# lrjconan/LanczosNetwork

Measured on NVIDIA H100. Metric: QM8 molecules/sec (forward), higher is better.
Workload: dtype f32

## Files before the change

lanczosnetwork_b200/csrc/spectral_conv_fused.cu:

```cuda
#include "tc_gemm.cuh"

namespace {

constexpr int KMAX = 32;
constexpr int GMAX = 32;
constexpr int RMAX = 128;
constexpr int EMAX = 16;
constexpr int FR = 8;

template <bool STAGE>
__global__ void __launch_bounds__(256)
graph_prepare_kernel(const float* __restrict__ L, const float* __restrict__ Q, int N, int E1, int K,
                     float* __restrict__ ell_val, uint8_t* __restrict__ ell_idx,
                     int32_t* __restrict__ ell_max, int32_t* __restrict__ gext, int binarize) {
  extern __shared__ __align__(16) float gp_smem[];
  __shared__ int s_max[EMAX];
  __shared__ int s_ext[2];
  __shared__ uint8_t cnt_s[256 * EMAX];
  const int b = blockIdx.x, tid = threadIdx.x;
  if (tid < EMAX) s_max[tid] = 0;
  if (tid < 2) s_ext[tid] = 0;
  const int64_t per = (int64_t)N * N * E1;
  const float* Lg = L + b * per;
  if (STAGE) {
// ... 476 lines not shown
  float* ring;
  tcg::PhaseTimer* ptm = nullptr;

  static __host__ __device__ constexpr size_t tables_bytes() { return (sizeof(Tables) + 15) & ~size_t(15); }

  __device__ SpectralPolicyT(const Params& p_, uint8_t* smem, int tid_)
      : p(p_), tid(tid_), r(tid_ & 127), N(p_.N), K(p_.K), S(p_.S), E1(p_.E1),
        H(p_.H), XP(x_pitch(p_.Din[0], p_.H)), Din(p_.Din[0]) {
    tb = reinterpret_cast<Tables*>(smem);
    Xs = reinterpret_cast<float*>(smem + tables_bytes());
    Qs = Xs + (size_t)RMAX * XP;
    Ev = Qs + (size_t)RMAX * K;
    Ei = reinterpret_cast<uint8_t*>(Ev + (size_t)p.LB * RMAX);
    ring = reinterpret_cast<float*>(tcg::a_ring(smem, kStagesB, kStagesA));
  }
  static size_t smem_fixed(int Din, int K, int H) {
    return (size_t)RMAX * x_pitch(Din, H) * 4 + (size_t)RMAX * K * 4 + tables_bytes() + 16;
  }
  static size_t ell_line_bytes() { return (size_t)RMAX * 5; }
  static size_t readout_bytes(int H, int P, int N) {
    const size_t P1 = (size_t)P + 1, PQ = (P1 + 3) / 4, yr = (RMAX + 1) * P1;
    return (4 * PQ * (H + 4) + yr + ((4 - (yr & 3)) & 3) + H) * 4 + (size_t)GMAX * N;
  }

  __device__ void build_tables(int m_tile) {
    const int lane = tid & 31;
    const int32_t* sc = schedule(p);
    const int s0 = __ldg(sc + 1 + m_tile), s1 = __ldg(sc + 2 + m_tile);
    const int ng = s1 - s0;
    int g = s0 + lane, n = 0, k = 0;
    if (lane < ng) {
      if (p.B >= 2) g = __ldg(sc + __ldg(sc) + 2 + s0 + lane);
      n = __ldg(p.gext + g * 2);
      k = __ldg(p.gext + g * 2 + 1);
    }
    const int nq = (n + 3) >> 2, kq = (k + 3) >> 2;
    int pn = n, pk = k, pq = nq, pz = kq;
#pragma unroll
    for (int o = 1; o < 32; o <<= 1) {
      const int a = __shfl_up_sync(0xffffffffu, pn, o), bq = __shfl_up_sync(0xffffffffu, pk, o);
      const int c = __shfl_up_sync(0xffffffffu, pq, o), d = __shfl_up_sync(0xffffffffu, pz, o);
      if (lane >= o) { pn += a; pk += bq; pq += c; pz += d; }
    }
    const int nb = pn - n, kb = pk - k, qb = pq - nq, zb = pz - kq;
    if (lane < ng) {
      tb->gid[lane] = g;
      tb->nbase[lane] = nb; tb->kbase[lane] = kb; tb->gn[lane] = n; tb->gk[lane] = k;
      for (int i = 0; i < n; ++i) { tb->row_g[nb + i] = (uint8_t)lane; tb->row_n[nb + i] = (uint8_t)i; }
      for (int i = 0; i < k; ++i) { tb->z_g[kb + i] = (uint8_t)lane; tb->z_k[kb + i] = (uint8_t)i; }
      for (int i = 0; i < nq; ++i) { tb->q_g[qb + i] = (uint8_t)lane; tb->q_n0[qb + i] = (uint8_t)(4 * i); }
      for (int i = 0; i < kq; ++i) { tb->zq_g[zb + i] = (uint8_t)lane; tb->zq_k0[zb + i] = (uint8_t)(4 * i); }
    }
    const int Rtot = __shfl_sync(0xffffffffu, pn, 31), Ztot = __shfl_sync(0xffffffffu, pk, 31);
    const int nquads = __shfl_sync(0xffffffffu, pq, 31), nzquads = __shfl_sync(0xffffffffu, pz, 31);
    int em[EMAX];
#pragma unroll
    for (int e = 0; e < EMAX; ++e)
      em[e] = (e < E1 && lane < ng) ? __ldg(p.ell_max + g * E1 + e) : 0;
#pragma unroll
    for (int e = 0; e < EMAX; ++e) {
      if (e < E1) {
        int m = em[e];
        if (lane < ng) tb->emax[lane][e] = (uint8_t)m;
#pragma unroll
        for (int o = 16; o > 0; o >>= 1) m = max(m, __shfl_xor_sync(0xffffffffu, m, o));
        if (lane == 0) tb->tmax_e[e] = m;
      }
    }
    __syncwarp();
    if (lane == 0) {
      tb->ng = ng; tb->Rtot = Rtot; tb->Ztot = Ztot; tb->nquads = nquads; tb->nzquads = nzquads;
      tb->nbase[ng] = Rtot; tb->kbase[ng] = Ztot;
      int left = p.LB, base = 0;
      for (int e = 0; e < E1; ++e) {
        const int c = min(tb->tmax_e[e], left);
        tb->cnt_e[e] = c; tb->base_e[e] = base;
        for (int t = 0; t < c; ++t) { tb->line_e[base + t] = (uint8_t)e; tb->line_t[base + t] = (uint8_t)t; }
        base += c; left -= c;
      }
      tb->nlines = base;
    }
  }

  __device__ void step_begin(int m_tile, int sub, int , tcg::PhaseTimer& tm) {
    tcg::producers_sync();
    const int layer = sub >> 1, step = sub & 1;
    if (step == 1 && S > 0) return;
    Din = p.Din[layer];
    const int warp = tid >> 5, lane = tid & 31;
    constexpr int NW = tcg::PRODUCER_THREADS / 32;
    const int dv = Din / 4;
    ptm = &tm;
    if (layer == 0) {
    if (warp == 0) build_tables(m_tile);
    tcg::producers_sync();
    tm.lap(16);
    const int Rtot = tb->Rtot;
    int64_t my_id = 0;
    if (!p.X && warp + lane * NW < Rtot) {
      const int row = warp + lane * NW;
      my_id = __ldg(p.node_ids + (int64_t)tb->gid[tb->row_g[row]] * N + tb->row_n[row]);
    }
    for (int row = warp, j = 0; row < Rtot; row += NW, ++j) {
      const int64_t src_row = (int64_t)tb->gid[tb->row_g[row]] * N + tb->row_n[row];
      const float* xsrc;
      if (p.X) {
        xsrc = p.X + src_row * Din;
      } else {
        int64_t id = __shfl_sync(0xffffffffu, my_id, j);
        id = id < 0 ? 0 : (id >= p.emb_rows ? p.emb_rows - 1 : id);
        xsrc = p.emb + id * Din;
      }
      float* xd = Xs + (size_t)row * XP;
      for (int q4 = lane; q4 < dv; q4 += 32) sm90::cp_async_16(xd + 4 * q4, xsrc + 4 * q4);
      const float* qsrc = p.Q + src_row * K;
      float* qd = Qs + (size_t)row * K;
      for (int k4 = lane; k4 < (K >> 2); k4 += 32) sm90::cp_async_16(qd + 4 * k4, qsrc + 4 * k4);
    }
    tm.lap(17);
    {
      constexpr int ELL_BATCH = 4;
      const int nlines = tb->nlines;
      for (int base = warp; base < nlines; base += NW * ELL_BATCH) {
        for (int r0 = 0; r0 < Rtot; r0 += 32) {
          const int rr = r0 + lane;
          float vv[ELL_BATCH];
          int ii[ELL_BATCH];
#pragma unroll
          for (int u = 0; u < ELL_BATCH; ++u) {
            const int line = base + u * NW;
            vv[u] = 0.f; ii[u] = 0;
            if (line < nlines && rr < Rtot) {
              const int e = tb->line_e[line], t = tb->line_t[line];
              const int g = tb->row_g[rr], n = tb->row_n[rr];
              if (t < tb->emax[g][e]) {
                const int64_t off = (((int64_t)tb->gid[g] * E1 + e) * N + t) * N + n;
                vv[u] = __ldg(p.ell_val + off);
                ii[u] = tb->nbase[g] + __ldg(p.ell_idx + off);
              }
            }
          }
#pragma unroll
          for (int u = 0; u < ELL_BATCH; ++u) {
            const int line = base + u * NW;
            if (line < nlines && rr < Rtot) {
              Ev[(size_t)line * RMAX + rr] = vv[u];
              Ei[(size_t)line * RMAX + rr] = (uint8_t)ii[u];
            }
          }
        }
      }
    }
    tm.lap(18);
    }
    const int Ztot = tb->Ztot;
#pragma unroll
    for (int i = 0; i < FR; ++i) fr[i] = 0.f;
    if (S > 0 && r < Ztot) {
      const float* f = p.coeff + layer * p.coeff_stride + ((int64_t)tb->gid[tb->z_g[r]] * K + tb->z_k[r]) * S;
#pragma unroll
      for (int i = 0; i < FR; ++i)
        if (i < S) fr[i] = __ldg(f + i);
    }
    tm.lap(0);
    sm90::cp_async_wait_all();
    tcg::producers_sync();
    tm.lap(1);
  }

  __device__ __forceinline__ void produce(int sub, int kb, float (&v)[32]) {
#pragma unroll
    for (int j = 0; j < 32; ++j) v[j] = 0.f;
    if (kLongScales && (sub & 1) == 0) {
      if (r >= tb->Ztot) return;
      const int s = kb % S;
      if (s == 0) {
        const int g = tb->z_g[r], n_g = tb->gn[g], nb = tb->nbase[g];
        const float* xs = Xs + (size_t)nb * XP + (kb / S) * tcg::BK;
        const float* qs = Qs + (size_t)nb * K + tb->z_k[r];
#pragma unroll
        for (int j = 0; j < tcg::BK; ++j) u[j] = 0.f;
#pragma unroll 2
        for (int n = 0; n < n_g; ++n) {
          const float q = qs[(size_t)n * K];
          const float4* x4 = reinterpret_cast<const float4*>(xs + (size_t)n * XP);
#pragma unroll
          for (int j = 0; j < 8; ++j) {
            const float4 t = x4[j];
            u[4 * j + 0] = fmaf(q, t.x, u[4 * j + 0]); u[4 * j + 1] = fmaf(q, t.y, u[4 * j + 1]);
            u[4 * j + 2] = fmaf(q, t.z, u[4 * j + 2]); u[4 * j + 3] = fmaf(q, t.w, u[4 * j + 3]);
          }
        }
      }
      float f = 0.f;
      if (S <= FR) {
#pragma unroll
        for (int i = 0; i < FR; ++i) f = (i == s) ? fr[i] : f;
      } else {
        f = __ldg(p.coeff + (sub >> 1) * p.coeff_stride + ((int64_t)tb->gid[tb->z_g[r]] * K + tb->z_k[r]) * S + s);
      }
#pragma unroll
      for (int j = 0; j < tcg::BK; ++j) v[j] = f * u[j];
      return;
    }
    const int j0 = kb * tcg::BK;
    const int c = j0 / Din, d0 = j0 - c * Din;
    if (r >= tb->Rtot) return;
    const int e = c;
    if constexpr (kMaxAgg) {
      produce_max(e, d0, v);
      return;
    }
    const float* xs = Xs + d0;
    const int ts = tb->cnt_e[e], tmax = tb->tmax_e[e];
    const float* ev = Ev + (size_t)tb->base_e[e] * RMAX + r;
    const uint8_t* ei = Ei + (size_t)tb->base_e[e] * RMAX + r;
#pragma unroll 2
    for (int t = 0; t < ts; ++t) {
      const float a = ev[t * RMAX];
      if (a == 0.f) continue;
      const int i = ei[t * RMAX];
      const float4* x4 = reinterpret_cast<const float4*>(xs + (size_t)i * XP);
#pragma unroll
      for (int q = 0; q < 8; ++q) {
        const float4 tt = x4[q];
        v[4 * q + 0] = fmaf(a, tt.x, v[4 * q + 0]);
        v[4 * q + 1] = fmaf(a, tt.y, v[4 * q + 1]);
        v[4 * q + 2] = fmaf(a, tt.z, v[4 * q + 2]);
        v[4 * q + 3] = fmaf(a, tt.w, v[4 * q + 3]);
      }
    }
    if (ts < tmax) {
      const int g = tb->row_g[r], n = tb->row_n[r];
      const int my = tb->emax[g][e], nb = tb->nbase[g];
      const int64_t off0 = (((int64_t)tb->gid[g] * E1 + e) * N) * N + n;
// ... 410 lines not shown
```

lanczosnetwork_b200/csrc/filter_mlp_chain.cu:

```cuda
#include "tc_gemm.cuh"

namespace {

constexpr int S0MAX = 8;

struct ChainPolicy {
  static constexpr int kStagesB = 2;
  static constexpr int kStagesA = 4;
  struct Params {
    const float* table;
    const int32_t* rowmap;
    const int32_t* nrows;
    const float* W_hi;
    const float* W_lo;
    const float* bias_all;
    float* coeff;
    int Rall, L, S, Hd;
    int dbg;
  };
  static __device__ __forceinline__ bool mma0(const Params& p) { return p.S > S0MAX; }
  static __device__ __forceinline__ int first_stage(const Params& p) { return mma0(p) ? 0 : 1; }
  static __device__ __forceinline__ int steps_per_item(const Params& p) { return mma0(p) ? 4 : 2; }
  static __device__ __forceinline__ int rows(const Params& p) { return p.nrows ? __ldg(p.nrows) : p.Rall; }
  static __device__ __forceinline__ int ntile(const Params& p) { return (rows(p) + tcg::BM - 1) / tcg::BM; }
  static __device__ __forceinline__ void item_range(const Params& p, int cta, int ncta, int& first,
                                                    int& count) {
    const int items = ntile(p) * p.L, base = items / ncta, rem = items % ncta;
    count = base + (cta < rem ? 1 : 0);
    first = cta * base + min(cta, rem);
  }
  static __device__ __forceinline__ int num_steps(const Params& p, int cta, int ncta) {
    int first, count;
    item_range(p, cta, ncta, first, count);
    return count * steps_per_item(p);
  }
  static __device__ __forceinline__ void decode(const Params& p, int cta, int ncta, int it,
                                                int& m_tile, int& sub) {
    const int per = steps_per_item(p), nt = ntile(p);
    int first, count;
    item_range(p, cta, ncta, first, count);
    const int item = first + it / per;
    m_tile = item % nt;
    sub = (item / nt) * 4 + first_stage(p) + it % per;
  }
  static __device__ __forceinline__ int num_kblocks(const Params& p, int sub) {
    return (sub & 3) == 0 ? 1 : p.Hd / tcg::BK;
  }
  static __device__ __forceinline__ int w_row0(const Params& p, int layer, int stage) {
    return layer * (3 * p.Hd + p.S) + stage * p.Hd;
  }
  static __device__ __forceinline__ void w_coords(const Params& p, int sub, int kb, int& col0, int& row0) {
    col0 = kb * tcg::BK;
    row0 = w_row0(p, sub >> 2, sub & 3);
  }
  static __device__ __forceinline__ bool operand_from_acc(const Params& p, int sub) {
    return (sub & 3) > first_stage(p);
  }
  static __device__ __forceinline__ float acc_operand(const Params&, const uint8_t* policy_smem, int sub, int col,
                                                      float x) {
    const float* bs = reinterpret_cast<const float*>(policy_smem) + BS_OFF;
    return fmaxf(x + bs[(sub & 3) * tcg::BN + col], 0.f);
  }

  const Params& p;
  const int tid, r;
  static constexpr int BS_OFF = 2 * tcg::BN * S0MAX;
  float* W1s;
  float* W3s;
  float* bs;
  float* b3s;
  int src, cur_layer;
  float tv[S0MAX];
  float o[S0MAX];

  static size_t smem_bytes() {
    return (BS_OFF + 3 * tcg::BN + S0MAX) * 4;
  }

  __device__ ChainPolicy(const Params& p_, uint8_t* smem, int tid_)
      : p(p_), tid(tid_), r(tid_ & 127), src(-1), cur_layer(-1) {
    W1s = reinterpret_cast<float*>(smem);
    W3s = W1s + tcg::BN * S0MAX;
    bs = W1s + BS_OFF;
    b3s = bs + 3 * tcg::BN;
  }

  __device__ void step_begin(int m_tile, int sub, int, tcg::PhaseTimer& tm) {
    const int layer = sub >> 2;
    if ((sub & 3) != first_stage(p)) return;
    const int i = m_tile * tcg::BM + r;
    src = i < rows(p) ? (p.rowmap ? __ldg(p.rowmap + i) : i) : -1;
    if (layer != cur_layer) {
      tcg::producers_sync();
      const int row0 = w_row0(p, layer, 0), row3 = w_row0(p, layer, 3);
      if (!mma0(p)) {
#pragma unroll 4
        for (int e = tid; e < p.Hd * S0MAX; e += tcg::PRODUCER_THREADS) {
          const int c = e / S0MAX, k = e - c * S0MAX;
          const int64_t o1 = (int64_t)(row0 + c) * p.Hd + k;
          W1s[e] = (k < p.S) ? __ldg(p.W_hi + o1) + __ldg(p.W_lo + o1) : 0.f;
          const int64_t o3 = (int64_t)(row3 + k) * p.Hd + c;
          W3s[e] = (k < p.S) ? __ldg(p.W_hi + o3) + __ldg(p.W_lo + o3) : 0.f;
        }
        if (tid < S0MAX) b3s[tid] = tid < p.S ? __ldg(p.bias_all + row3 + tid) : 0.f;
      }
      for (int e = tid; e < 3 * tcg::BN; e += tcg::PRODUCER_THREADS) {
        const int st = e / tcg::BN, c = e - st * tcg::BN;
        bs[e] = c < p.Hd ? __ldg(p.bias_all + row0 + st * p.Hd + c) : 0.f;
      }
      tcg::producers_sync();
      cur_layer = layer;
      tm.lap(1);
    }
    if (mma0(p)) return;
#pragma unroll
    for (int k = 0; k < S0MAX; ++k)
      tv[k] = (src >= 0 && k < p.S) ? __ldg(p.table + (int64_t)src * p.S + k) : 0.f;
  }

  __device__ __forceinline__ void produce(int sub, int kb, float (&v)[32]) {
    if ((sub & 3) == 0) {
#pragma unroll
      for (int j = 0; j < 32; ++j)
        v[j] = (src >= 0 && j < p.S) ? __ldg(p.table + (int64_t)src * p.S + j) : 0.f;
      return;
    }
#pragma unroll
    for (int j = 0; j < 32; ++j) {
      const int c = kb * tcg::BK + j;
      const float4* wr = reinterpret_cast<const float4*>(W1s + c * S0MAX);
      const float4 wa = wr[0], wb = wr[1];
      float a = bs[c];
      a = fmaf(tv[0], wa.x, a); a = fmaf(tv[1], wa.y, a); a = fmaf(tv[2], wa.z, a); a = fmaf(tv[3], wa.w, a);
      a = fmaf(tv[4], wb.x, a); a = fmaf(tv[5], wb.y, a); a = fmaf(tv[6], wb.z, a); a = fmaf(tv[7], wb.w, a);
      v[j] = fmaxf(a, 0.f);
    }
  }
  __device__ __forceinline__ void pre_epilogue(int) {}
  __device__ __forceinline__ void post_epilogue(int) {}

  __device__ __forceinline__ void store(int sub, int col, const float (&x)[tcg::EW]) {
    const int layer = sub >> 2, stage = sub & 3;
    if (stage == 3) {
      if (src < 0 || col >= p.S) return;
      const float* bias = p.bias_all + w_row0(p, layer, stage);
      float* dst = p.coeff + ((int64_t)layer * p.Rall + src) * p.S;
#pragma unroll
      for (int j = 0; j < tcg::EW; ++j)
        if (col + j < p.S) dst[col + j] = x[j] + __ldg(bias + col + j);
      return;
    }
    if (col >= p.Hd) return;
    const float* b2 = bs + 2 * tcg::BN;
    if (col == 0) {
#pragma unroll
      for (int s = 0; s < S0MAX; ++s) o[s] = 0.f;
    }
#pragma unroll
    for (int j = 0; j < tcg::EW; ++j) {
      const float y = fmaxf(x[j] + b2[col + j], 0.f);
      const float4* wr = reinterpret_cast<const float4*>(W3s + (col + j) * S0MAX);
      const float4 wa = wr[0], wb = wr[1];
      o[0] = fmaf(y, wa.x, o[0]); o[1] = fmaf(y, wa.y, o[1]);
      o[2] = fmaf(y, wa.z, o[2]); o[3] = fmaf(y, wa.w, o[3]);
      o[4] = fmaf(y, wb.x, o[4]); o[5] = fmaf(y, wb.y, o[5]);
      o[6] = fmaf(y, wb.z, o[6]); o[7] = fmaf(y, wb.w, o[7]);
    }
    if (col + tcg::EW < p.Hd || src < 0) return;
    float* dst = p.coeff + ((int64_t)layer * p.Rall + src) * p.S;
#pragma unroll
    for (int s = 0; s < S0MAX; ++s)
      if (s < p.S) dst[s] = o[s] + b3s[s];
  }
};

__global__ void __launch_bounds__(1024)
ritz_rowmap_kernel(const int32_t* __restrict__ gext, int B, int K, int32_t* __restrict__ rowmap,
                   int32_t* __restrict__ nrows) {
  __shared__ int warp_sums[32];
  __shared__ int running;
  const int tid = threadIdx.x, lane = tid & 31, warp = tid >> 5;
  if (tid == 0) running = 0;
  __syncthreads();
  for (int b0 = 0; b0 < B; b0 += 1024) {
    const int b = b0 + tid;
    int k = (b < B) ? min(gext[b * 2 + 1], K) : 0;
    int incl = k;
#pragma unroll
    for (int o = 1; o < 32; o <<= 1) {
      const int t = __shfl_up_sync(0xffffffffu, incl, o);
      if (lane >= o) incl += t;
    }
    if (lane == 31) warp_sums[warp] = incl;
    __syncthreads();
    if (warp == 0) {
      int w = warp_sums[lane], wi = w;
#pragma unroll
      for (int o = 1; o < 32; o <<= 1) {
        const int t = __shfl_up_sync(0xffffffffu, wi, o);
        if (lane >= o) wi += t;
      }
      warp_sums[lane] = wi - w;
    }
    __syncthreads();
    const int base = running + warp_sums[warp] + incl - k;
    for (int i = 0; i < k; ++i) rowmap[base + i] = b * K + i;
    __syncthreads();
    if (tid == 1023) running = base + k;
    __syncthreads();
  }
  if (tid == 0) nrows[0] = running;
}

}

extern "C" {

int lnb_ritz_rowmap(lnb_stream_t stream, const int32_t* gext, int B, int K, int32_t* rowmap,
                    int32_t* nrows) {
  LNB_REQUIRE(gext && rowmap && nrows, "ritz_rowmap: null pointer");
  LNB_REQUIRE(B >= 0 && K >= 1, "ritz_rowmap: bad dims");
  ritz_rowmap_kernel<<<1, 1024, 0, (cudaStream_t)stream>>>(gext, B, K, rowmap, nrows);
  lnb::count_launch();
  return lnb::finish_launch("ritz_rowmap");
}

int lnb_ritz_filter_mlp(lnb_stream_t stream, const float* table, const int32_t* rowmap,
                        const int32_t* nrows, const float* W_hi, const float* W_lo,
                        const float* bias_all, int Rall, int L, int S, int Hd, float* coeff) {
  LNB_REQUIRE(table && W_hi && W_lo && bias_all && coeff, "ritz_filter_mlp: null pointer");
  LNB_REQUIRE((rowmap == nullptr) == (nrows == nullptr), "ritz_filter_mlp: rowmap and nrows go together");
  LNB_REQUIRE(Rall >= 0 && L >= 1 && S >= 1 && Hd >= 1, "ritz_filter_mlp: bad dims");
  if (S > 32 || Hd % 32 != 0 || Hd > tcg::BN) {
    lnb::set_err("ritz_filter_mlp: unsupported shape S=%d hidden=%d (needs S<=32, hidden%%32==0, hidden<=128)", S, Hd);
    return LNB_ERR_UNSUPPORTED;
  }
  if (Rall == 0) return LNB_OK;
  const size_t smem = tcg::core_smem(ChainPolicy::kStagesB, ChainPolicy::kStagesA) + 1024 + ChainPolicy::smem_bytes();
  ChainPolicy::Params p{table, rowmap, nrows, W_hi, W_lo, bias_all, coeff, Rall, L, S, Hd, tcg::debug_flags()};
  return tcg::launch<ChainPolicy>(stream, W_hi, W_lo, L * (3 * Hd + S), Hd, smem, lnb::ceil_div(Rall, tcg::BM) * L, p,
                                  "ritz_filter_mlp");
}

}
```

lanczosnetwork_b200/csrc/tc_gemm.cuh:

```cuda
#pragma once
#include "common.cuh"
#include "sm90.cuh"
#include <stdlib.h>
#include <type_traits>

namespace tcg {

constexpr int BM = 128, BN = 128, BK = 32;
constexpr int NGROUPS = 1;
constexpr int TILE_B_BYTES = BN * BK * 4;
constexpr int STAGE_B_BYTES = 2 * TILE_B_BYTES;
constexpr int TILE_A_BYTES = BM * BK * 4;
constexpr int STAGE_A_BYTES = 2 * TILE_A_BYTES;
constexpr int EW = 16;
constexpr int PRODUCER_THREADS = 128 * NGROUPS;
constexpr int CONSUMER_WARP0 = PRODUCER_THREADS / 32;
constexpr int CONSUMER_THREADS = 256;
constexpr int THREADS = PRODUCER_THREADS + CONSUMER_THREADS;
constexpr int MAX_B_STAGES = 6, MAX_A_STAGES = 4;
__host__ __device__ constexpr int core_smem(int stages_b, int stages_a) {
  return stages_b * STAGE_B_BYTES + stages_a * STAGE_A_BYTES + 256;
}
__host__ __device__ constexpr int pass_cols(int stages_a) {
  return stages_a * STAGE_A_BYTES / (BM * 4) < BN ? stages_a * STAGE_A_BYTES / (BM * 4) : BN;
}

__device__ __forceinline__ uint8_t* a_ring(uint8_t* policy_smem, int stages_b, int stages_a) {
  return policy_smem - core_smem(stages_b, stages_a) + stages_b * STAGE_B_BYTES;
}

struct Core {
  uint8_t* Bst;
  uint8_t* Ast;
  uint64_t* b_full;
  uint64_t* b_empty;
  uint64_t* a_full;
  uint64_t* a_empty;
  uint64_t* stg_full;
  uint64_t* stg_empty;
  uint64_t* kept_read;
};

__device__ __forceinline__ Core carve(uint8_t* base, int stages_b, int stages_a) {
  Core c;
  c.Bst = base;
  c.Ast = base + stages_b * STAGE_B_BYTES;
  uint64_t* bars = reinterpret_cast<uint64_t*>(c.Ast + stages_a * STAGE_A_BYTES);
  c.b_full = bars;
  c.b_empty = c.b_full + MAX_B_STAGES;
  c.a_full = c.b_empty + MAX_B_STAGES;
  c.a_empty = c.a_full + MAX_A_STAGES;
  c.stg_full = c.a_empty + MAX_A_STAGES;
  c.stg_empty = c.stg_full + 1;
  c.kept_read = c.stg_empty + 1;
  return c;
}

__device__ unsigned long long* g_prof = nullptr;

struct PhaseTimer {
  unsigned long long* buf;
  long long t0;
  __device__ __forceinline__ void start(int cta, int tid) {
    buf = (tid == 0 && g_prof) ? g_prof + cta * 32 : nullptr;
    if (buf) t0 = clock64();
  }
  __device__ __forceinline__ void start_if(int cta, bool owner) {
    buf = (owner && g_prof) ? g_prof + cta * 32 : nullptr;
    if (buf) t0 = clock64();
  }
  __device__ __forceinline__ void lap(int slot) {
    if (buf) { long long t = clock64(); atomicAdd(&buf[slot], (unsigned long long)(t - t0)); t0 = t; }
  }
};

__device__ __forceinline__ void producers_sync() {
  asm volatile("bar.sync 1, %0;" ::"n"(PRODUCER_THREADS) : "memory");
}
__device__ __forceinline__ void consumers_sync() {
  asm volatile("bar.sync 2, %0;" ::"n"(CONSUMER_THREADS) : "memory");
}

__device__ __forceinline__ int stg_index(int row, int col, int pw) {
  return row * pw + ((((col >> 2) ^ row) & (pw / 4 - 1)) << 2) + (col & 3);
}

template <class P, class = void> struct HasAccInit : std::false_type {};
template <class P> struct HasAccInit<P, std::void_t<decltype(&P::acc_init)>> : std::true_type {};
template <class P, class = void> struct HasOperandFromAcc : std::false_type {};
template <class P> struct HasOperandFromAcc<P, std::void_t<decltype(&P::operand_from_acc)>> : std::true_type {};

template <class Policy>
__device__ __forceinline__ bool next_from_acc(const typename Policy::Params& p, int cta, int ncta, int it,
                                              int nsteps, int& nkb_next) {
  if (it + 1 >= nsteps) return false;
  int m_tile, sub;
  Policy::decode(p, cta, ncta, it + 1, m_tile, sub);
  nkb_next = Policy::num_kblocks(p, sub);
  return Policy::operand_from_acc(p, sub);
}

constexpr int SKIP_MMA = 2;
constexpr int SKIP_TMA = 4;

template <class Policy, int kSkip>
__device__ __forceinline__ void tc_gemm_body(const CUtensorMap& map_hi, const CUtensorMap& map_lo,
                                             const typename Policy::Params& p) {
  extern __shared__ __align__(16) uint8_t smem_raw[];
  const uint32_t pad = (1024u - (sm90::smem_u32(smem_raw) & 1023u)) & 1023u;
  uint8_t* base = smem_raw + pad;
  constexpr int SB = Policy::kStagesB, SA = Policy::kStagesA;
  static_assert(SB >= 1 && SB <= MAX_B_STAGES && SA >= 1 && SA <= MAX_A_STAGES, "ring depths");
  constexpr int PW = pass_cols(SA);
  constexpr int NPASS = BN / PW;
  constexpr bool kAccInit = HasAccInit<Policy>::value;
  static_assert(!kAccInit || NPASS == 1, "a drain kept in the A ring must fit it in one pass");
  constexpr bool kOpAcc = HasOperandFromAcc<Policy>::value;
  constexpr bool kQueue = !kAccInit;
  static_assert(!kOpAcc || SA * BK >= BN, "an operand written from the accumulators needs one A stage per k-block");
  Core c = carve(base, SB, SA);
  uint8_t* policy_smem = base + core_smem(SB, SA);
  float* stg = reinterpret_cast<float*>(c.Ast);

  const int tid = threadIdx.x, warp = tid >> 5, lane = tid & 31;
  const int role = __shfl_sync(0xffffffffu, tid / 128, 0);
  const int cta = blockIdx.x, ncta = gridDim.x;
  const int nsteps = __shfl_sync(0xffffffffu, Policy::num_steps(p, cta, ncta), 0);
  unsigned long long prof_ns0 = 0;
  long long prof_c0 = 0;
  if (tid == 0 && g_prof) {
    asm volatile("mov.u64 %0, %globaltimer;" : "=l"(prof_ns0));
    prof_c0 = clock64();
  }

  if (warp == CONSUMER_WARP0 && lane == 0) {
    sm90::tma_prefetch_desc(&map_hi);
    sm90::tma_prefetch_desc(&map_lo);
    for (int s = 0; s < SB; ++s) {
      sm90::mbar_init(&c.b_full[s], 1);
      sm90::mbar_init(&c.b_empty[s], CONSUMER_THREADS / 32);
    }
    for (int s = 0; s < SA; ++s) {
      sm90::mbar_init(&c.a_full[s], PRODUCER_THREADS);
      sm90::mbar_init(&c.a_empty[s], CONSUMER_THREADS / 32);
    }
    sm90::mbar_init(c.stg_full, CONSUMER_THREADS);
    sm90::mbar_init(c.stg_empty, PRODUCER_THREADS);
    sm90::mbar_init(c.kept_read, CONSUMER_THREADS / 32);
    sm90::fence_barrier_init();
  }
  __syncthreads();

  if (role == 0) {
    const int r = tid & 127;
    Policy pol(p, policy_smem, tid);
    uint32_t cnt = 0;
    uint32_t npass = 0;
    uint32_t nkept = 0;
    bool after_kept = false;
    for (int it = 0; it < nsteps; ++it) {
      int m_tile, sub;
      Policy::decode(p, cta, ncta, it, m_tile, sub);
      int nkb = Policy::num_kblocks(p, sub);
      bool kept = false, to_acc = false;
      if constexpr (kAccInit) kept = Policy::drain_kept(p, sub);
      if constexpr (kOpAcc) {
        if (Policy::operand_from_acc(p, sub)) nkb = 0;
        int nkb_next;
        to_acc = next_from_acc<Policy>(p, cta, ncta, it, nsteps, nkb_next);
      }
      PhaseTimer tm;
      tm.start(cta, tid);
      pol.step_begin(m_tile, sub, 0, tm);
      for (int kb = 0; kb < nkb; ++kb, ++cnt) {
        float v[32];
        if (!(p.dbg & 8)) pol.produce(sub, kb, v);
        const uint32_t sa = cnt % SA;
        if (kAccInit && kb == 0 && after_kept) {
          sm90::mbar_wait(c.kept_read, nkept & 1u);
          ++nkept;
        }
        sm90::mbar_wait(&c.a_empty[sa], ((cnt / SA) & 1u) ^ 1u);
        if (!(p.dbg & 1)) {
          uint8_t* hi = c.Ast + sa * STAGE_A_BYTES + r * 128;
#pragma unroll
          for (int j = 0; j < 8; ++j) {
            uint4 h, l;
            h.x = sm90::tf32_rna_bits(v[4 * j + 0]); h.y = sm90::tf32_rna_bits(v[4 * j + 1]);
            h.z = sm90::tf32_rna_bits(v[4 * j + 2]); h.w = sm90::tf32_rna_bits(v[4 * j + 3]);
            l.x = sm90::tf32_rna_bits(v[4 * j + 0] - __uint_as_float(h.x));
            l.y = sm90::tf32_rna_bits(v[4 * j + 1] - __uint_as_float(h.y));
            l.z = sm90::tf32_rna_bits(v[4 * j + 2] - __uint_as_float(h.z));
            l.w = sm90::tf32_rna_bits(v[4 * j + 3] - __uint_as_float(h.w));
            const int off = (j ^ (r & 7)) * 16;
            *reinterpret_cast<uint4*>(hi + off) = h;
            *reinterpret_cast<uint4*>(hi + TILE_A_BYTES + off) = l;
          }
        }
        sm90::fence_proxy_async();
        sm90::mbar_arrive(&c.a_full[sa]);
      }
      tm.lap((sub & 1) ? 8 : 3);
      pol.pre_epilogue(sub);
      tm.lap(4);
#pragma unroll 1
      for (int q = 0; q < (kept || to_acc ? 0 : NPASS); ++q, ++npass) {
        sm90::mbar_wait(c.stg_full, npass & 1u);
        if (q == 0) tm.lap((sub & 1) ? 9 : 5);
#pragma unroll 1
        for (int col = q * PW; col < (q + 1) * PW; col += EW) {
          float x[EW];
#pragma unroll
          for (int j = 0; j < EW; j += 4) {
            const float4 t = *reinterpret_cast<const float4*>(stg + stg_index(r, col - q * PW + j, PW));
            x[j] = t.x; x[j + 1] = t.y; x[j + 2] = t.z; x[j + 3] = t.w;
          }
          pol.store(sub, col, x);
        }
        sm90::mbar_arrive(c.stg_empty);
      }
      tm.lap(7);
      producers_sync();
      pol.post_epilogue(sub);
      tm.lap(10);
      after_kept = kept;
    }
  } else {
    const int wg = role - 1;
    const int wq = warp & 3;
    float d[128];
    uint32_t cnt = 0, npass = 0;
    uint32_t nacc = 0;
    bool after_kept = false;
    const int row0 = wg * 64 + wq * 16 + (lane >> 2), cl = 2 * (lane & 3);
    const bool w_issuer = warp == CONSUMER_WARP0;
    int l_it = 0, l_kb = 0, l_nkb = -1, l_sub = 0;
    uint32_t l_cnt = 0;
    auto load_next = [&]() {
      while (l_it < nsteps) {
        if (l_nkb < 0) {
          int mt;
          Policy::decode(p, cta, ncta, l_it, mt, l_sub);
          l_nkb = Policy::num_kblocks(p, l_sub);
        }
        if (l_kb < l_nkb) break;
        ++l_it; l_kb = 0; l_nkb = -1;
      }
      if (l_it >= nsteps) return;
      int col0, row0;
      Policy::w_coords(p, l_sub, l_kb, col0, row0);
      const uint32_t st = l_cnt % SB;
      sm90::mbar_wait_uniform(&c.b_empty[st], ((l_cnt / SB) & 1u) ^ 1u);
      uint8_t* dst = c.Bst + st * STAGE_B_BYTES;
      sm90::tma_load_2d_pair_elected<(kSkip & SKIP_TMA) != 0>(w_issuer, &c.b_full[st], STAGE_B_BYTES, dst, &map_hi,
                                                               dst + TILE_B_BYTES, &map_lo, col0, row0);
      ++l_kb; ++l_cnt;
    };
    auto release = [&](uint32_t sb_rel, bool a_stage, uint32_t sa_rel) {
      sm90::mbar_arrive_pred(&c.a_empty[sa_rel], a_stage && lane == 0);
      sm90::mbar_arrive_pred(&c.b_empty[sb_rel], lane == 0);
      load_next();
    };
    for (int i = 0; i < SB; ++i) load_next();
    for (int it = 0; it < nsteps; ++it) {
      int m_tile, sub;
      Policy::decode(p, cta, ncta, it, m_tile, sub);
      const int nkb = Policy::num_kblocks(p, sub);
      bool kept = false, from_acc = false, to_acc = false;
      int nkb_next = 0;
      if constexpr (kOpAcc) {
        from_acc = Policy::operand_from_acc(p, sub);
        to_acc = next_from_acc<Policy>(p, cta, ncta, it, nsteps, nkb_next);
      }
      if constexpr (kAccInit) {
        kept = Policy::drain_kept(p, sub);
        sm90::wgmma_fence_operand(d);
        if (!Policy::acc_init(p, policy_smem, stg, sub, row0, cl, d)) {
#pragma unroll
          for (int i = 0; i < 128; ++i) d[i] = 0.f;
        }
        if (after_kept) {
          __syncwarp();
          if (lane == 0) sm90::mbar_arrive(c.kept_read);
        }
      } else {
#pragma unroll
        for (int i = 0; i < 128; ++i) d[i] = 0.f;
      }
      sm90::wgmma_fence_operand(d);
      for (int kb = 0; kb < nkb; ++kb, ++cnt) {
        const uint32_t acnt = cnt - nacc;
        const uint32_t sb = cnt % SB, sa = from_acc ? (uint32_t)kb : acnt % SA;
        sm90::mbar_wait_uniform(&c.b_full[sb], (cnt / SB) & 1u);
        if (!from_acc) sm90::mbar_wait_uniform(&c.a_full[sa], (acnt / SA) & 1u);
        if constexpr (!(kSkip & SKIP_MMA)) {
          const uint32_t a_hi = sm90::smem_u32(c.Ast + sa * STAGE_A_BYTES) + wg * 64 * 128;
          const uint32_t a_lo = a_hi + TILE_A_BYTES;
          const uint32_t b = sm90::smem_u32(c.Bst + sb * STAGE_B_BYTES);
          sm90::wgmma_fence_operand(d);
          sm90::wgmma_fence();
#pragma unroll
          for (int k = 0; k < BK / 8; ++k) {
            const uint64_t ah = sm90::wgmma_desc_kmajor_sw128(a_hi + 32 * k);
            const uint64_t wh = sm90::wgmma_desc_kmajor_sw128(b + 32 * k);
            sm90::wgmma_n128(d, ah, wh, 1u);
            sm90::wgmma_n128_hi(d, ah, sm90::wgmma_desc_kmajor_sw128(b + TILE_B_BYTES + 32 * k), 1u);
            sm90::wgmma_n128_hi(d, sm90::wgmma_desc_kmajor_sw128(a_lo + 32 * k), wh, 1u);
          }
          sm90::wgmma_commit();
          if constexpr (kQueue) sm90::wgmma_wait_one();
          else sm90::wgmma_wait_all();
          sm90::wgmma_fence_operand(d);
        }
        if constexpr (kQueue) {
          if (kb > 0) release((cnt - 1) % SB, !from_acc, from_acc ? (uint32_t)(kb - 1) : (acnt - 1) % SA);
        } else {
          release(sb, !from_acc, sa);
        }
      }
      if constexpr (!(kSkip & SKIP_MMA)) {
        sm90::wgmma_wait_all();
        sm90::wgmma_fence_operand(d);
      }
      if (kQueue && nkb > 0)
        release((cnt - 1) % SB, !from_acc, from_acc ? (uint32_t)(nkb - 1) : (cnt - nacc - 1) % SA);
      if (from_acc) nacc += nkb;
      PhaseTimer ctm;
      if (to_acc) ctm.start_if(cta, tid == PRODUCER_THREADS);
      consumers_sync();
      if (to_acc) {
        if constexpr (kOpAcc) {
#pragma unroll
          for (int i = 0; i < 64; i += 2) {
            const int col = 8 * (i / 4) + cl, row = row0 + 8 * ((i / 2) % 2), kb = i / 16;
            if (kb < nkb_next) {
              const float y0 = Policy::acc_operand(p, policy_smem, sub, col, d[i] + d[i + 64]);
              const float y1 = Policy::acc_operand(p, policy_smem, sub, col + 1, d[i + 1] + d[i + 65]);
              uint2 h, l;
              h.x = sm90::tf32_rna_bits(y0); h.y = sm90::tf32_rna_bits(y1);
              l.x = sm90::tf32_rna_bits(y0 - __uint_as_float(h.x));
              l.y = sm90::tf32_rna_bits(y1 - __uint_as_float(h.y));
              uint8_t* dst = c.Ast + kb * STAGE_A_BYTES + row * 128 + (((((col & 31) >> 2) ^ row) & 7) << 4) +
                             (col & 3) * 4;
              *reinterpret_cast<uint2*>(dst) = h;
              *reinterpret_cast<uint2*>(dst + TILE_A_BYTES) = l;
            }
          }
          sm90::fence_proxy_async();
          consumers_sync();
          ctm.lap(14);
        }
      } else {
#pragma unroll
        for (int q = 0; q < NPASS; ++q, npass += kept ? 0 : 1) {
          if (!kept) sm90::mbar_wait(c.stg_empty, (npass & 1u) ^ 1u);
#pragma unroll
          for (int i = 0; i < 64; i += 2) {
            const int col = 8 * (i / 4) + cl, row = row0 + 8 * ((i / 2) % 2);
            if (col >= q * PW && col < (q + 1) * PW)
              *reinterpret_cast<float2*>(stg + stg_index(row, col - q * PW, PW)) =
                  make_float2(d[i] + d[i + 64], d[i + 1] + d[i + 65]);
          }
          if (!kept) sm90::mbar_arrive(c.stg_full);
        }
      }
      if (kept) consumers_sync();
      after_kept = kept;
    }
  }

  __syncthreads();
  if (tid == 0 && g_prof) {
    unsigned long long ns1;
    asm volatile("mov.u64 %0, %globaltimer;" : "=l"(ns1));
    atomicAdd(&g_prof[cta * 32 + 11], ns1 - prof_ns0);
    atomicAdd(&g_prof[cta * 32 + 12], (unsigned long long)(clock64() - prof_c0));
    g_prof[cta * 32 + 13] = prof_ns0;
  }
}

template <class Policy>
__global__ void __launch_bounds__(THREADS, 1)
tc_gemm_kernel(const __grid_constant__ CUtensorMap map_hi,
               const __grid_constant__ CUtensorMap map_lo, const typename Policy::Params p) {
  tc_gemm_body<Policy, 0>(map_hi, map_lo, p);
}

template <class Policy, int kSkip>
__global__ void __launch_bounds__(THREADS, 1)
tc_gemm_probe_kernel(const __grid_constant__ CUtensorMap map_hi,
                     const __grid_constant__ CUtensorMap map_lo, const typename Policy::Params p) {
  tc_gemm_body<Policy, kSkip>(map_hi, map_lo, p);
}

__device__ __forceinline__ void store_row_chunk(float* orow, int ncols, const float* bias, bool relu,
                                                int col, const float (&x)[EW]) {
  if (orow == nullptr || col >= ncols) return;
  const bool vec_ok = (reinterpret_cast<uintptr_t>(orow + col) & 15) == 0;
#pragma unroll
  for (int j = 0; j < EW; j += 4) {
    float o[4];
#pragma unroll
    for (int u = 0; u < 4; ++u) {
      const int n = col + j + u;
      float y = x[j + u];
      if (n < ncols) {
        if (bias) y += __ldg(bias + n);
        if (relu) y = fmaxf(y, 0.f);
      }
      o[u] = y;
    }
    if (vec_ok && col + j + 3 < ncols) {
      *reinterpret_cast<float4*>(orow + col + j) = make_float4(o[0], o[1], o[2], o[3]);
    } else {
#pragma unroll
      for (int u = 0; u < 4; ++u)
        if (col + j + u < ncols) orow[col + j + u] = o[u];
    }
  }
}

typedef CUresult (*EncodeTiledFn)(CUtensorMap*, CUtensorMapDataType, cuuint32_t, void*,
                                  const cuuint64_t*, const cuuint64_t*, const cuuint32_t*,
                                  const cuuint32_t*, CUtensorMapInterleave, CUtensorMapSwizzle,
                                  CUtensorMapL2promotion, CUtensorMapFloatOOBfill);

inline EncodeTiledFn get_encode_fn() {
  static EncodeTiledFn fn = nullptr;
  if (!fn) {
    void* ptr = nullptr;
    cudaDriverEntryPointQueryResult q;
    if (cudaGetDriverEntryPoint("cuTensorMapEncodeTiled", &ptr, cudaEnableDefault, &q) == cudaSuccess &&
        q == cudaDriverEntryPointSuccess)
      fn = reinterpret_cast<EncodeTiledFn>(ptr);
  }
  return fn;
}

inline int make_weight_map(CUtensorMap* map, const float* W, int rows, int cols, const char* who,
                           int box_rows = BN) {
  EncodeTiledFn enc = get_encode_fn();
  if (!enc) { lnb::set_err("%s: cuTensorMapEncodeTiled unavailable", who); return LNB_ERR_UNSUPPORTED; }
  cuuint64_t gdim[2] = {(cuuint64_t)cols, (cuuint64_t)rows};
// ... 60 lines not shown
```

Before: 1.070 million.

## Defer ELL staging to second step and use per-row thread mapping

When S > 0, the ELL value/index staging for layer 0 moves out of the first step's begin and into the begin of the second sub-step. This is meant to take it off the critical path before the first GEMM step can start. X/Q row loads and ELL staging now map one producer thread per row instead of one warp per row with lanes striding columns. That removes the shuffle-broadcast of node ids and the per-element table lookups, but each thread now issues many serial cp.async/loads and global accesses are no longer coalesced across lanes.

```diff
diff --git a/lanczosnetwork_b200/csrc/spectral_conv_fused.cu b/lanczosnetwork_b200/csrc/spectral_conv_fused.cu
--- a/lanczosnetwork_b200/csrc/spectral_conv_fused.cu
+++ b/lanczosnetwork_b200/csrc/spectral_conv_fused.cu
@@ -582,13 +582,52 @@
     }
   }
 
+  __device__ void stage_ell_lines() {
+    if (r >= tb->Rtot) return;
+    constexpr int ELL_BATCH = 16;
+    const int my_g = tb->row_g[r], my_n = tb->row_n[r];
+    const int nlines = tb->nlines, nb = tb->nbase[my_g];
+    const uint8_t* em = tb->emax[my_g];
+    const int64_t off0 = ((int64_t)tb->gid[my_g] * E1 * N) * N + my_n;
+    for (int base = 0; base < nlines; base += ELL_BATCH) {
+      float vv[ELL_BATCH];
+      int ii[ELL_BATCH];
+#pragma unroll
+      for (int u = 0; u < ELL_BATCH; ++u) {
+        const int line = base + u;
+        vv[u] = 0.f; ii[u] = 0;
+        if (line < nlines) {
+          const int e = tb->line_e[line], t = tb->line_t[line];
+          if (t < em[e]) {
+            const int64_t off = off0 + ((int64_t)e * N + t) * N;
+            vv[u] = __ldg(p.ell_val + off);
+            ii[u] = nb + __ldg(p.ell_idx + off);
+          }
+        }
+      }
+#pragma unroll
+      for (int u = 0; u < ELL_BATCH; ++u) {
+        const int line = base + u;
+        if (line < nlines) {
+          Ev[(size_t)line * RMAX + r] = vv[u];
+          Ei[(size_t)line * RMAX + r] = (uint8_t)ii[u];
+        }
+      }
+    }
+  }
+
   __device__ void step_begin(int m_tile, int sub, int , tcg::PhaseTimer& tm) {
     tcg::producers_sync();
     const int layer = sub >> 1, step = sub & 1;
-    if (step == 1 && S > 0) return;
+    if (step == 1 && S > 0) {
+      if (layer == 0) {
+        stage_ell_lines();
+        tm.lap(18);
+      }
+      return;
+    }
     Din = p.Din[layer];
-    const int warp = tid >> 5, lane = tid & 31;
-    constexpr int NW = tcg::PRODUCER_THREADS / 32;
+    const int warp = tid >> 5;
     const int dv = Din / 4;
     ptm = &tm;
     if (layer == 0) {
@@ -596,61 +635,27 @@
     tcg::producers_sync();
     tm.lap(16);
     const int Rtot = tb->Rtot;
-    int64_t my_id = 0;
-    if (!p.X && warp + lane * NW < Rtot) {
-      const int row = warp + lane * NW;
-      my_id = __ldg(p.node_ids + (int64_t)tb->gid[tb->row_g[row]] * N + tb->row_n[row]);
-    }
-    for (int row = warp, j = 0; row < Rtot; row += NW, ++j) {
-      const int64_t src_row = (int64_t)tb->gid[tb->row_g[row]] * N + tb->row_n[row];
+    const int my_g = r < Rtot ? tb->row_g[r] : 0, my_n = r < Rtot ? tb->row_n[r] : 0;
+    const int my_gid = tb->gid[my_g];
+    if (r < Rtot) {
+      const int64_t src_row = (int64_t)my_gid * N + my_n;
       const float* xsrc;
       if (p.X) {
         xsrc = p.X + src_row * Din;
       } else {
-        int64_t id = __shfl_sync(0xffffffffu, my_id, j);
+        int64_t id = __ldg(p.node_ids + src_row);
         id = id < 0 ? 0 : (id >= p.emb_rows ? p.emb_rows - 1 : id);
         xsrc = p.emb + id * Din;
       }
-      float* xd = Xs + (size_t)row * XP;
-      for (int q4 = lane; q4 < dv; q4 += 32) sm90::cp_async_16(xd + 4 * q4, xsrc + 4 * q4);
+      float* xd = Xs + (size_t)r * XP;
+#pragma unroll 4
+      for (int q4 = 0; q4 < dv; ++q4) sm90::cp_async_16(xd + 4 * q4, xsrc + 4 * q4);
       const float* qsrc = p.Q + src_row * K;
-      float* qd = Qs + (size_t)row * K;
-      for (int k4 = lane; k4 < (K >> 2); k4 += 32) sm90::cp_async_16(qd + 4 * k4, qsrc + 4 * k4);
+      float* qd = Qs + (size_t)r * K;
+      for (int k4 = 0; k4 < (K >> 2); ++k4) sm90::cp_async_16(qd + 4 * k4, qsrc + 4 * k4);
     }
     tm.lap(17);
-    {
-      constexpr int ELL_BATCH = 4;
-      const int nlines = tb->nlines;
-      for (int base = warp; base < nlines; base += NW * ELL_BATCH) {
-        for (int r0 = 0; r0 < Rtot; r0 += 32) {
-          const int rr = r0 + lane;
-          float vv[ELL_BATCH];
-          int ii[ELL_BATCH];
-#pragma unroll
-          for (int u = 0; u < ELL_BATCH; ++u) {
-            const int line = base + u * NW;
-            vv[u] = 0.f; ii[u] = 0;
-            if (line < nlines && rr < Rtot) {
-              const int e = tb->line_e[line], t = tb->line_t[line];
-              const int g = tb->row_g[rr], n = tb->row_n[rr];
-              if (t < tb->emax[g][e]) {
-                const int64_t off = (((int64_t)tb->gid[g] * E1 + e) * N + t) * N + n;
-                vv[u] = __ldg(p.ell_val + off);
-                ii[u] = tb->nbase[g] + __ldg(p.ell_idx + off);
-              }
-            }
-          }
-#pragma unroll
-          for (int u = 0; u < ELL_BATCH; ++u) {
-            const int line = base + u * NW;
-            if (line < nlines && rr < Rtot) {
-              Ev[(size_t)line * RMAX + rr] = vv[u];
-              Ei[(size_t)line * RMAX + rr] = (uint8_t)ii[u];
-            }
-          }
-        }
-      }
-    }
+    if (S == 0) stage_ell_lines();
     tm.lap(18);
     }
     const int Ztot = tb->Ztot;
```

Measured after the change: 1.083 million (median of 6 runs). 1.2% higher.

## Drain epilogue through upper A stages so producers prefetch next tile early

Applied to the files above, without the earlier changes.

Moves the accumulator drain buffer above a reserved low A-ring region (kDrainStage=2), shrinking the A ring to two stages for this policy. Producers can then stage and write the next tile's first A blocks while the consumer-drain epilogue of the current tile is still being read. A new low_free barrier signals when the lower stages are free, and weight staging is split so the stage-3 weights are loaded only after the pending output has been written. The cost is a shallower A ring and more barrier traffic, with a risk of ordering bugs.

```diff
diff --git a/lanczosnetwork_b200/csrc/filter_mlp_chain.cu b/lanczosnetwork_b200/csrc/filter_mlp_chain.cu
--- a/lanczosnetwork_b200/csrc/filter_mlp_chain.cu
+++ b/lanczosnetwork_b200/csrc/filter_mlp_chain.cu
@@ -61,6 +61,7 @@
     const float* bs = reinterpret_cast<const float*>(policy_smem) + BS_OFF;
     return fmaxf(x + bs[(sub & 3) * tcg::BN + col], 0.f);
   }
+  static constexpr int kDrainStage = 2;
 
   const Params& p;
   const int tid, r;
@@ -70,6 +71,9 @@
   float* bs;
   float* b3s;
   int src, cur_layer;
+  int src_out;
+  bool out_pending;
+  int rest_layer;
   float tv[S0MAX];
   float o[S0MAX];
 
@@ -78,11 +82,32 @@
   }
 
   __device__ ChainPolicy(const Params& p_, uint8_t* smem, int tid_)
-      : p(p_), tid(tid_), r(tid_ & 127), src(-1), cur_layer(-1) {
+      : p(p_), tid(tid_), r(tid_ & 127), src(-1), cur_layer(-1), src_out(-1), out_pending(false), rest_layer(-1) {
     W1s = reinterpret_cast<float*>(smem);
     W3s = W1s + tcg::BN * S0MAX;
     bs = W1s + BS_OFF;
     b3s = bs + 3 * tcg::BN;
+  }
+
+  __device__ void stage_layer(int layer, bool first, bool rest) {
+    tcg::producers_sync();
+    const int row0 = w_row0(p, layer, 0), row3 = w_row0(p, layer, 3);
+    if (!mma0(p)) {
+#pragma unroll 4
+      for (int e = tid; e < p.Hd * S0MAX; e += tcg::PRODUCER_THREADS) {
+        const int c = e / S0MAX, k = e - c * S0MAX;
+        const int64_t o1 = (int64_t)(row0 + c) * p.Hd + k;
+        if (first) W1s[e] = (k < p.S) ? __ldg(p.W_hi + o1) + __ldg(p.W_lo + o1) : 0.f;
+        const int64_t o3 = (int64_t)(row3 + k) * p.Hd + c;
+        if (rest) W3s[e] = (k < p.S) ? __ldg(p.W_hi + o3) + __ldg(p.W_lo + o3) : 0.f;
+      }
+      if (rest && tid < S0MAX) b3s[tid] = tid < p.S ? __ldg(p.bias_all + row3 + tid) : 0.f;
+    }
+    for (int e = tid; e < 3 * tcg::BN; e += tcg::PRODUCER_THREADS) {
+      const int st = e / tcg::BN, c = e - st * tcg::BN;
+      if (st == 0 ? first : rest) bs[e] = c < p.Hd ? __ldg(p.bias_all + row0 + st * p.Hd + c) : 0.f;
+    }
+    tcg::producers_sync();
   }
 
   __device__ void step_begin(int m_tile, int sub, int, tcg::PhaseTimer& tm) {
@@ -91,24 +116,8 @@
     const int i = m_tile * tcg::BM + r;
     src = i < rows(p) ? (p.rowmap ? __ldg(p.rowmap + i) : i) : -1;
     if (layer != cur_layer) {
-      tcg::producers_sync();
-      const int row0 = w_row0(p, layer, 0), row3 = w_row0(p, layer, 3);
-      if (!mma0(p)) {
-#pragma unroll 4
-        for (int e = tid; e < p.Hd * S0MAX; e += tcg::PRODUCER_THREADS) {
-          const int c = e / S0MAX, k = e - c * S0MAX;
-          const int64_t o1 = (int64_t)(row0 + c) * p.Hd + k;
-          W1s[e] = (k < p.S) ? __ldg(p.W_hi + o1) + __ldg(p.W_lo + o1) : 0.f;
-          const int64_t o3 = (int64_t)(row3 + k) * p.Hd + c;
-          W3s[e] = (k < p.S) ? __ldg(p.W_hi + o3) + __ldg(p.W_lo + o3) : 0.f;
-        }
-        if (tid < S0MAX) b3s[tid] = tid < p.S ? __ldg(p.bias_all + row3 + tid) : 0.f;
-      }
-      for (int e = tid; e < 3 * tcg::BN; e += tcg::PRODUCER_THREADS) {
-        const int st = e / tcg::BN, c = e - st * tcg::BN;
-        bs[e] = c < p.Hd ? __ldg(p.bias_all + row0 + st * p.Hd + c) : 0.f;
-      }
-      tcg::producers_sync();
+      stage_layer(layer, !(out_pending && mma0(p)), !out_pending);
+      rest_layer = out_pending ? layer : -1;
       cur_layer = layer;
       tm.lap(1);
     }
@@ -136,15 +145,24 @@
       v[j] = fmaxf(a, 0.f);
     }
   }
-  __device__ __forceinline__ void pre_epilogue(int) {}
-  __device__ __forceinline__ void post_epilogue(int) {}
+  __device__ __forceinline__ void pre_epilogue(int) {
+    src_out = src;
+    out_pending = true;
+  }
+  __device__ void post_epilogue(int) {
+    out_pending = false;
+    if (rest_layer >= 0) {
+      stage_layer(rest_layer, mma0(p), true);
+      rest_layer = -1;
+    }
+  }
 
   __device__ __forceinline__ void store(int sub, int col, const float (&x)[tcg::EW]) {
     const int layer = sub >> 2, stage = sub & 3;
     if (stage == 3) {
-      if (src < 0 || col >= p.S) return;
+      if (src_out < 0 || col >= p.S) return;
       const float* bias = p.bias_all + w_row0(p, layer, stage);
-      float* dst = p.coeff + ((int64_t)layer * p.Rall + src) * p.S;
+      float* dst = p.coeff + ((int64_t)layer * p.Rall + src_out) * p.S;
 #pragma unroll
       for (int j = 0; j < tcg::EW; ++j)
         if (col + j < p.S) dst[col + j] = x[j] + __ldg(bias + col + j);
@@ -166,8 +184,8 @@
       o[4] = fmaf(y, wb.x, o[4]); o[5] = fmaf(y, wb.y, o[5]);
       o[6] = fmaf(y, wb.z, o[6]); o[7] = fmaf(y, wb.w, o[7]);
     }
-    if (col + tcg::EW < p.Hd || src < 0) return;
-    float* dst = p.coeff + ((int64_t)layer * p.Rall + src) * p.S;
+    if (col + tcg::EW < p.Hd || src_out < 0) return;
+    float* dst = p.coeff + ((int64_t)layer * p.Rall + src_out) * p.S;
 #pragma unroll
     for (int s = 0; s < S0MAX; ++s)
       if (s < p.S) dst[s] = o[s] + b3s[s];
diff --git a/lanczosnetwork_b200/csrc/tc_gemm.cuh b/lanczosnetwork_b200/csrc/tc_gemm.cuh
--- a/lanczosnetwork_b200/csrc/tc_gemm.cuh
+++ b/lanczosnetwork_b200/csrc/tc_gemm.cuh
@@ -39,6 +39,7 @@
   uint64_t* stg_full;
   uint64_t* stg_empty;
   uint64_t* kept_read;
+  uint64_t* low_free;
 };
 
 __device__ __forceinline__ Core carve(uint8_t* base, int stages_b, int stages_a) {
@@ -53,6 +54,7 @@
   c.stg_full = c.a_empty + MAX_A_STAGES;
   c.stg_empty = c.stg_full + 1;
   c.kept_read = c.stg_empty + 1;
+  c.low_free = c.kept_read + 1;
   return c;
 }
 
@@ -89,6 +91,27 @@
 template <class P> struct HasAccInit<P, std::void_t<decltype(&P::acc_init)>> : std::true_type {};
 template <class P, class = void> struct HasOperandFromAcc : std::false_type {};
 template <class P> struct HasOperandFromAcc<P, std::void_t<decltype(&P::operand_from_acc)>> : std::true_type {};
+template <class P, class = void> struct DrainStage : std::integral_constant<int, 0> {};
+template <class P> struct DrainStage<P, std::void_t<decltype(P::kDrainStage)>>
+    : std::integral_constant<int, P::kDrainStage> {};
+template <class P> constexpr int kDrainStageOf = DrainStage<P>::value;
+template <class P> constexpr int kRingA = kDrainStageOf<P> > 0 ? kDrainStageOf<P> : P::kStagesA;
+
+__device__ __forceinline__ void write_a_row(uint8_t* hi, int r, const float (&v)[32]) {
+#pragma unroll
+  for (int j = 0; j < 8; ++j) {
+    uint4 h, l;
+    h.x = sm90::tf32_rna_bits(v[4 * j + 0]); h.y = sm90::tf32_rna_bits(v[4 * j + 1]);
+    h.z = sm90::tf32_rna_bits(v[4 * j + 2]); h.w = sm90::tf32_rna_bits(v[4 * j + 3]);
+    l.x = sm90::tf32_rna_bits(v[4 * j + 0] - __uint_as_float(h.x));
+    l.y = sm90::tf32_rna_bits(v[4 * j + 1] - __uint_as_float(h.y));
+    l.z = sm90::tf32_rna_bits(v[4 * j + 2] - __uint_as_float(h.z));
+    l.w = sm90::tf32_rna_bits(v[4 * j + 3] - __uint_as_float(h.w));
+    const int off = (j ^ (r & 7)) * 16;
+    *reinterpret_cast<uint4*>(hi + off) = h;
+    *reinterpret_cast<uint4*>(hi + TILE_A_BYTES + off) = l;
+  }
+}
 
 template <class Policy>
 __device__ __forceinline__ bool next_from_acc(const typename Policy::Params& p, int cta, int ncta, int it,
@@ -118,6 +141,9 @@
   constexpr bool kOpAcc = HasOperandFromAcc<Policy>::value;
   constexpr bool kQueue = !kAccInit;
   static_assert(!kOpAcc || SA * BK >= BN, "an operand written from the accumulators needs one A stage per k-block");
+  constexpr bool kDrainAt = kDrainStageOf<Policy> > 0;
+  static_assert(!kDrainAt || (NPASS == 1 && kQueue && kOpAcc && (SA - kDrainStageOf<Policy>) * STAGE_A_BYTES >= BM * BN * 4),
+                "a drain above stage 0 needs one pass in the stages above it, one group queued and operand_from_acc");
   Core c = carve(base, SB, SA);
   uint8_t* policy_smem = base + core_smem(SB, SA);
   float* stg = reinterpret_cast<float*>(c.Ast);
@@ -147,6 +173,7 @@
     sm90::mbar_init(c.stg_full, CONSUMER_THREADS);
     sm90::mbar_init(c.stg_empty, PRODUCER_THREADS);
     sm90::mbar_init(c.kept_read, CONSUMER_THREADS / 32);
+    if constexpr (kDrainAt) sm90::mbar_init(c.low_free, CONSUMER_THREADS / 32);
     sm90::fence_barrier_init();
   }
   __syncthreads();
@@ -158,6 +185,9 @@
     uint32_t npass = 0;
     uint32_t nkept = 0;
     bool after_kept = false;
+    uint32_t nlow = 0;
+    int early = 0;
+    bool begun = false;
     for (int it = 0; it < nsteps; ++it) {
       int m_tile, sub;
       Policy::decode(p, cta, ncta, it, m_tile, sub);
@@ -169,40 +199,54 @@
         int nkb_next;
         to_acc = next_from_acc<Policy>(p, cta, ncta, it, nsteps, nkb_next);
       }
+      const int s0 = kept || to_acc ? 0 : kDrainStageOf<Policy>;
       PhaseTimer tm;
       tm.start(cta, tid);
-      pol.step_begin(m_tile, sub, 0, tm);
-      for (int kb = 0; kb < nkb; ++kb, ++cnt) {
+      if (!begun) pol.step_begin(m_tile, sub, 0, tm);
+      for (int kb = early; kb < nkb; ++kb, ++cnt) {
         float v[32];
         if (!(p.dbg & 8)) pol.produce(sub, kb, v);
-        const uint32_t sa = cnt % SA;
+        const uint32_t sa = cnt % kRingA<Policy>;
         if (kAccInit && kb == 0 && after_kept) {
           sm90::mbar_wait(c.kept_read, nkept & 1u);
           ++nkept;
         }
-        sm90::mbar_wait(&c.a_empty[sa], ((cnt / SA) & 1u) ^ 1u);
-        if (!(p.dbg & 1)) {
-          uint8_t* hi = c.Ast + sa * STAGE_A_BYTES + r * 128;
-#pragma unroll
-          for (int j = 0; j < 8; ++j) {
-            uint4 h, l;
-            h.x = sm90::tf32_rna_bits(v[4 * j + 0]); h.y = sm90::tf32_rna_bits(v[4 * j + 1]);
-            h.z = sm90::tf32_rna_bits(v[4 * j + 2]); h.w = sm90::tf32_rna_bits(v[4 * j + 3]);
-            l.x = sm90::tf32_rna_bits(v[4 * j + 0] - __uint_as_float(h.x));
-            l.y = sm90::tf32_rna_bits(v[4 * j + 1] - __uint_as_float(h.y));
-            l.z = sm90::tf32_rna_bits(v[4 * j + 2] - __uint_as_float(h.z));
-            l.w = sm90::tf32_rna_bits(v[4 * j + 3] - __uint_as_float(h.w));
-            const int off = (j ^ (r & 7)) * 16;
-            *reinterpret_cast<uint4*>(hi + off) = h;
-            *reinterpret_cast<uint4*>(hi + TILE_A_BYTES + off) = l;
-          }
-        }
+        sm90::mbar_wait(&c.a_empty[sa], ((cnt / kRingA<Policy>) & 1u) ^ 1u);
+        if (!(p.dbg & 1)) write_a_row(c.Ast + sa * STAGE_A_BYTES + r * 128, r, v);
         sm90::fence_proxy_async();
         sm90::mbar_arrive(&c.a_full[sa]);
       }
       tm.lap((sub & 1) ? 8 : 3);
       pol.pre_epilogue(sub);
       tm.lap(4);
+      if constexpr (kDrainAt) {
+        early = 0;
+        begun = false;
+        if (s0 > 0 && it + 1 < nsteps) {
+          int m_next, sub_next;
+          Policy::decode(p, cta, ncta, it + 1, m_next, sub_next);
+          bool produced = true;
+          if constexpr (kOpAcc) produced = !Policy::operand_from_acc(p, sub_next);
+          if (produced) {
+            const int nkb_next = Policy::num_kblocks(p, sub_next);
+            pol.step_begin(m_next, sub_next, 0, tm);
+            begun = true;
+            for (; early < nkb_next; ++early, ++cnt) {
+              float v[32];
+              if (!(p.dbg & 8)) pol.produce(sub_next, early, v);
+              const uint32_t sa = cnt % kRingA<Policy>;
+              if (early == 0) sm90::mbar_wait(c.low_free, nlow & 1u);
+              sm90::mbar_wait(&c.a_empty[sa], ((cnt / kRingA<Policy>) & 1u) ^ 1u);
+              if (!(p.dbg & 1)) write_a_row(c.Ast + sa * STAGE_A_BYTES + r * 128, r, v);
+              sm90::fence_proxy_async();
+              sm90::mbar_arrive(&c.a_full[sa]);
+            }
+            tm.lap(6);
+          }
+        }
+        if (s0 > 0) ++nlow;
+      }
+      const float* drain = stg + s0 * (STAGE_A_BYTES / 4);
 #pragma unroll 1
       for (int q = 0; q < (kept || to_acc ? 0 : NPASS); ++q, ++npass) {
         sm90::mbar_wait(c.stg_full, npass & 1u);
@@ -212,16 +256,17 @@
           float x[EW];
 #pragma unroll
           for (int j = 0; j < EW; j += 4) {
-            const float4 t = *reinterpret_cast<const float4*>(stg + stg_index(r, col - q * PW + j, PW));
+            const float4 t = *reinterpret_cast<const float4*>(drain + stg_index(r, col - q * PW + j, PW));
             x[j] = t.x; x[j + 1] = t.y; x[j + 2] = t.z; x[j + 3] = t.w;
           }
           pol.store(sub, col, x);
         }
-        sm90::mbar_arrive(c.stg_empty);
+        if constexpr (!kDrainAt) sm90::mbar_arrive(c.stg_empty);
       }
       tm.lap(7);
       producers_sync();
       pol.post_epilogue(sub);
+      if constexpr (kDrainAt) if (s0 > 0) sm90::mbar_arrive(c.stg_empty);
       tm.lap(10);
       after_kept = kept;
     }
@@ -272,6 +317,7 @@
         from_acc = Policy::operand_from_acc(p, sub);
         to_acc = next_from_acc<Policy>(p, cta, ncta, it, nsteps, nkb_next);
       }
+      const int s0 = to_acc ? 0 : kDrainStageOf<Policy>;
       if constexpr (kAccInit) {
         kept = Policy::drain_kept(p, sub);
         sm90::wgmma_fence_operand(d);
@@ -290,9 +336,9 @@
       sm90::wgmma_fence_operand(d);
       for (int kb = 0; kb < nkb; ++kb, ++cnt) {
         const uint32_t acnt = cnt - nacc;
-        const uint32_t sb = cnt % SB, sa = from_acc ? (uint32_t)kb : acnt % SA;
+        const uint32_t sb = cnt % SB, sa = from_acc ? (uint32_t)kb : acnt % kRingA<Policy>;
         sm90::mbar_wait_uniform(&c.b_full[sb], (cnt / SB) & 1u);
-        if (!from_acc) sm90::mbar_wait_uniform(&c.a_full[sa], (acnt / SA) & 1u);
+        if (!from_acc) sm90::mbar_wait_uniform(&c.a_full[sa], (acnt / kRingA<Policy>) & 1u);
         if constexpr (!(kSkip & SKIP_MMA)) {
           const uint32_t a_hi = sm90::smem_u32(c.Ast + sa * STAGE_A_BYTES) + wg * 64 * 128;
           const uint32_t a_lo = a_hi + TILE_A_BYTES;
@@ -313,7 +359,8 @@
           sm90::wgmma_fence_operand(d);
         }
         if constexpr (kQueue) {
-          if (kb > 0) release((cnt - 1) % SB, !from_acc, from_acc ? (uint32_t)(kb - 1) : (acnt - 1) % SA);
+          if (kb > 0) release((cnt - 1) % SB, !from_acc, from_acc ? (uint32_t)(kb - 1) : (acnt - 1) % kRingA<Policy>);
+          if constexpr (kDrainAt) sm90::mbar_arrive_pred(c.low_free, s0 > 0 && kb == s0 && lane == 0);
         } else {
           release(sb, !from_acc, sa);
         }
@@ -323,13 +370,15 @@
         sm90::wgmma_fence_operand(d);
       }
       if (kQueue && nkb > 0)
-        release((cnt - 1) % SB, !from_acc, from_acc ? (uint32_t)(nkb - 1) : (cnt - nacc - 1) % SA);
+        release((cnt - 1) % SB, !from_acc, from_acc ? (uint32_t)(nkb - 1) : (cnt - nacc - 1) % kRingA<Policy>);
+      if constexpr (kDrainAt) sm90::mbar_arrive_pred(c.low_free, s0 > 0 && nkb <= s0 && lane == 0);
       if (from_acc) nacc += nkb;
       PhaseTimer ctm;
       if (to_acc) ctm.start_if(cta, tid == PRODUCER_THREADS);
       consumers_sync();
       if (to_acc) {
         if constexpr (kOpAcc) {
+          if constexpr (kDrainAt) sm90::mbar_wait(c.stg_empty, (npass & 1u) ^ 1u);
 #pragma unroll
           for (int i = 0; i < 64; i += 2) {
             const int col = 8 * (i / 4) + cl, row = row0 + 8 * ((i / 2) % 2), kb = i / 16;
@@ -351,6 +400,7 @@
           ctm.lap(14);
         }
       } else {
+        float* drain = stg + s0 * (STAGE_A_BYTES / 4);
 #pragma unroll
         for (int q = 0; q < NPASS; ++q, npass += kept ? 0 : 1) {
           if (!kept) sm90::mbar_wait(c.stg_empty, (npass & 1u) ^ 1u);
@@ -358,7 +408,7 @@
           for (int i = 0; i < 64; i += 2) {
             const int col = 8 * (i / 4) + cl, row = row0 + 8 * ((i / 2) % 2);
             if (col >= q * PW && col < (q + 1) * PW)
-              *reinterpret_cast<float2*>(stg + stg_index(row, col - q * PW, PW)) =
+              *reinterpret_cast<float2*>(drain + stg_index(row, col - q * PW, PW)) =
                   make_float2(d[i] + d[i + 64], d[i + 1] + d[i + 65]);
           }
           if (!kept) sm90::mbar_arrive(c.stg_full);
```

Result: no change. 1.063 million before, 1.079 million after (median of 6 runs) (+1.5%).
